# Fadi987/PL-BERT

Hardware: AMD Instinct MI355X
Metric: phoneme-tokens/sec (higher is better)
Workload: dtype bf16; 1 GPU; PL-BERT masked-phoneme training step (fwd+loss+bwd+allreduce+AdamW), ALBERT hidden 768 / 12 shared layers / FFN 2048 / 12 heads, seq_len 512, batch 32 per GPU; global_batch=32, seq_len=512, parallelism=dp1

## Files before the change

plbert_amd/_lib.py:

```python
from __future__ import annotations

import ctypes as C
import os

import torch

HERE = os.path.dirname(os.path.abspath(__file__))
LIB_PATH = os.environ.get("PLBERT_HIP_LIB") or os.path.join(HERE, "libplbert_hip.so")

PLB_PARAM_NAMES = [
    "encoder.embeddings.word_embeddings.weight",
    "encoder.embeddings.position_embeddings.weight",
    "encoder.embeddings.token_type_embeddings.weight",
    "encoder.embeddings.LayerNorm.weight",
    "encoder.embeddings.LayerNorm.bias",
    "encoder.encoder.embedding_hidden_mapping_in.weight",
    "encoder.encoder.embedding_hidden_mapping_in.bias",
    "encoder.encoder.albert_layer_groups.0.albert_layers.0.full_layer_layer_norm.weight",
    "encoder.encoder.albert_layer_groups.0.albert_layers.0.full_layer_layer_norm.bias",
    "encoder.encoder.albert_layer_groups.0.albert_layers.0.attention.query.weight",
    "encoder.encoder.albert_layer_groups.0.albert_layers.0.attention.key.weight",
    "encoder.encoder.albert_layer_groups.0.albert_layers.0.attention.value.weight",
    "encoder.encoder.albert_layer_groups.0.albert_layers.0.attention.query.bias",
    "encoder.encoder.albert_layer_groups.0.albert_layers.0.attention.key.bias",
# ... 41 lines not shown
        ("ln_eps", C.c_float), ("ln_xchg", C.c_void_p), ("ln_err", C.c_void_p), ("ln_fault", C.c_int),
    ]


class PlbGemmTN(C.Structure):
    _fields_ = [
        ("A", C.c_void_p), ("lda", C.c_int), ("Ncols", C.c_int), ("B", C.c_void_p), ("ldb", C.c_int),
        ("Mtot", C.c_int), ("N", C.c_int), ("K", C.c_int), ("rows_per_split", C.c_int), ("splits", C.c_int),
        ("slab", C.c_void_p), ("deq_a", C.c_void_p), ("deq_b", C.c_void_p),
    ]


class PlbAttn(C.Structure):
    _fields_ = [
        ("qkv", C.c_void_p), ("ldqkv", C.c_int), ("lengths", C.c_void_p),
        ("B", C.c_int), ("S", C.c_int), ("NH", C.c_int), ("H", C.c_int), ("scale", C.c_float),
        ("ctx", C.c_void_p), ("ldctx", C.c_int), ("lse", C.c_void_p),
        ("dctx", C.c_void_p), ("lddctx", C.c_int), ("delta", C.c_void_p), ("dqkv", C.c_void_p), ("lddqkv", C.c_int),
        ("colpart", C.c_void_p), ("colpart_accumulate", C.c_int),
        ("ctx8", C.c_void_p), ("ldctx8", C.c_int), ("ctx_scale", C.c_void_p), ("ctx_amax", C.c_void_p),
        ("dqkv8", C.c_void_p), ("lddqkv8", C.c_int), ("dqkv_scale", C.c_void_p), ("dqkv_amax", C.c_void_p),
        ("qoff", C.c_void_p), ("q", C.c_void_p), ("ldq", C.c_int), ("nq_total", C.c_int), ("dq", C.c_void_p), ("lddq", C.c_int),
        ("dq8", C.c_void_p), ("lddq8", C.c_int),
        ("row_start", C.c_void_p),
    ]


class PlbEmbed(C.Structure):
    _fields_ = [
        ("ids", C.c_void_p), ("T", C.c_int), ("S", C.c_int), ("E", C.c_int), ("V", C.c_int),
        ("word", C.c_void_p), ("pos", C.c_void_p), ("type0", C.c_void_p), ("gamma", C.c_void_p), ("beta", C.c_void_p),
        ("eps", C.c_float), ("out", C.c_void_p), ("ldo", C.c_int), ("dout", C.c_void_p), ("lddo", C.c_int),
        ("dx", C.c_void_p), ("dword", C.c_void_p), ("dpos", C.c_void_p), ("partials", C.c_void_p), ("nblocks", C.c_int),
        ("row_start", C.c_void_p), ("lengths", C.c_void_p), ("B", C.c_int), ("fill_slots", C.c_int),
    ]


class PlbPacking(C.Structure):
    _fields_ = [("row_start", C.c_void_p), ("rows", C.c_int32), ("used", C.c_int32)]


class PlbLayerOutputs(C.Structure):
    _fields_ = [("hidden_states", C.c_void_p), ("attentions", C.c_void_p)]


class PlbMaskedReport(C.Structure):
    _fields_ = [
        ("pred", C.c_void_p), ("rank", C.c_void_p), ("nll", C.c_void_p), ("topk_ids", C.c_void_p), ("topk_logprob", C.c_void_p),
        ("logits", C.c_void_p), ("sample_loss", C.c_void_p), ("sample_top1", C.c_void_p), ("sample_topk", C.c_void_p),
        ("totals", C.c_void_p), ("token_totals", C.c_void_p),
    ]


class PlbTokenReport(C.Structure):
    _fields_ = [
        ("topk_ids", C.c_void_p), ("topk_logprob", C.c_void_p), ("lse", C.c_void_p), ("target_logprob", C.c_void_p),
        ("target_pos", C.c_void_p), ("logits", C.c_void_p), ("totals", C.c_void_p),
    ]


class PlbLayerNorm(C.Structure):
    _fields_ = [
        ("x", C.c_void_p), ("ldx", C.c_int), ("gamma", C.c_void_p), ("beta", C.c_void_p), ("eps", C.c_float),
        ("y", C.c_void_p), ("ldy", C.c_int), ("mean", C.c_void_p), ("rstd", C.c_void_p),
        ("T", C.c_int), ("H", C.c_int), ("Tzero", C.c_int),
        ("dy", C.c_void_p), ("lddy", C.c_int), ("dx", C.c_void_p), ("lddx", C.c_int),
# ... 231 lines not shown
```

plbert_amd/csrc/embed.hip:

```cpp
#include "common.h"
#include "plbert_kernels.h"
#include "row_common.h"

namespace {
template <bool BWD>
__global__ __launch_bounds__(256) void embed_kernel(PlbEmbed p) {
  const int lane = threadIdx.x & 63, wave = threadIdx.x >> 6;
  const int E = p.E;
  const int c = lane * 4;
  const bool act = c < E;
  float4 g4 = make_float4(0, 0, 0, 0), b4 = g4, ty = g4;
  if (act) {
    g4 = *(const float4*)(p.gamma + c);
    b4 = *(const float4*)(p.beta + c);
    ty = *(const float4*)(p.type0 + c);
  }
  float dg[4] = {0, 0, 0, 0}, db[4] = {0, 0, 0, 0};
  const float invE = 1.0f / (float)E;
  for (int t = blockIdx.x * 4 + wave; t < p.T; t += gridDim.x * 4) {
    int src = t, s = 0;
    if (p.row_start) {
      int b;
      const bool owned = packed_locate(p.row_start, p.lengths, p.B, p.S, t, &b, &s);
      if (!owned && !(!BWD && p.fill_slots && s < p.S && t < p.row_start[b + 1])) {
// ... 52 lines not shown
    __shared__ float red[4][2][256];
    if (act) {
#pragma unroll
      for (int j = 0; j < 4; ++j) { red[wave][0][c + j] = dg[j]; red[wave][1][c + j] = db[j]; }
    }
    __syncthreads();
    for (int i = threadIdx.x; i < 2 * E; i += 256) {
      const int which = i / E, col = i % E;
      p.partials[(size_t)blockIdx.x * 2 * E + i] =
          red[0][which][col] + red[1][which][col] + red[2][which][col] + red[3][which][col];
    }
  }
}
}
extern "C" int plb_launch_embed_fwd(const PlbEmbed* p, hipStream_t stream) {
  if (p->E % 4 || p->E > 256 || p->T <= 0) return 1;
  if (p->row_start && (!p->lengths || p->B < 1)) return 1;
  int blocks = (p->T + 3) / 4; if (blocks > 2048) blocks = 2048;
  ProfScope ps(PLB_K_EMBED_FWD, stream, 0, (double)p->T * (8 + 2.0 * p->E));
  hipLaunchKernelGGL((embed_kernel<false>), dim3(blocks), dim3(256), 0, stream, *p);
  return LAUNCH_OK();
}
extern "C" int plb_launch_embed_bwd(const PlbEmbed* p, hipStream_t stream) {
  if (p->E % 4 || p->E > 256 || p->T <= 0 || p->nblocks <= 0) return 1;
  if (p->row_start && (!p->lengths || p->B < 1)) return 1;
  ProfScope ps(PLB_K_EMBED_BWD, stream, 0, (double)p->T * (8 + 2.0 * p->E + 8.0 * p->E));
  hipLaunchKernelGGL((embed_kernel<true>), dim3(p->nblocks), dim3(256), 0, stream, *p);
  return LAUNCH_OK();
}

namespace {
constexpr int EMB_CHUNK = 32768;
template <bool PACKED>
__global__ __launch_bounds__(256) void embed_scatter_kernel(PlbEmbed p, int P) {
  extern __shared__ int list[];
  __shared__ int wcnt[4];
  __shared__ float4 part[256];
  const int E = p.E, T = PACKED ? p.B * p.S : p.T;
  const int row = blockIdx.x;
  const int EQ = E >> 2;
  const int q = threadIdx.x % EQ, grp = threadIdx.x / EQ, ngrp = 256 / EQ;
  float4 s = make_float4(0.f, 0.f, 0.f, 0.f);
  auto add = [&](int t) {
    const float4 v = *(const float4*)(p.dx + (size_t)t * E + 4 * q);
    s.x += v.x; s.y += v.y; s.z += v.z; s.w += v.w;
  };
  if (row < p.V) {
    const int w = threadIdx.x >> 6, lane = threadIdx.x & 63;
    const int chunk = T < EMB_CHUNK ? T : EMB_CHUNK;
    const int cap = (chunk + 3) / 4 + 64;
    for (int c0 = 0; c0 < T && row != 0; c0 += EMB_CHUNK) {
      const int c1 = c0 + EMB_CHUNK < T ? c0 + EMB_CHUNK : T;
      int cnt = 0;
      for (int t0 = c0 + w * 64; t0 < c1; t0 += 256) {
        const int t = t0 + lane;
        bool hit = t < c1 && p.ids[t] == row;
        int trow = t;
        if (PACKED && hit) {
          const int b = t / p.S, sp = t - b * p.S;
          hit = sp < max(p.lengths[b], 1);
          trow = p.row_start[b] + sp;
        }
        const unsigned long long m = __builtin_amdgcn_ballot_w64(hit);
        if (hit) list[w * cap + cnt + __builtin_popcountll(m & ((1ull << lane) - 1ull))] = trow;
        cnt += __builtin_popcountll(m);
      }
      if (lane == 0) wcnt[w] = cnt;
      __syncthreads();
      for (int ww = 0; ww < 4; ++ww) {
        const int n = wcnt[ww];
        const int* l = list + ww * cap;
        int i = grp;
        for (; i + 7 * ngrp < n; i += 8 * ngrp) {
          float4 v[8];
#pragma unroll
          for (int k = 0; k < 8; ++k) v[k] = *(const float4*)(p.dx + (size_t)l[i + k * ngrp] * E + 4 * q);
          s.x += ((v[0].x + v[1].x) + (v[2].x + v[3].x)) + ((v[4].x + v[5].x) + (v[6].x + v[7].x));
          s.y += ((v[0].y + v[1].y) + (v[2].y + v[3].y)) + ((v[4].y + v[5].y) + (v[6].y + v[7].y));
          s.z += ((v[0].z + v[1].z) + (v[2].z + v[3].z)) + ((v[4].z + v[5].z) + (v[6].z + v[7].z));
          s.w += ((v[0].w + v[1].w) + (v[2].w + v[3].w)) + ((v[4].w + v[5].w) + (v[6].w + v[7].w));
        }
        for (; i + 3 * ngrp < n; i += 4 * ngrp) {
          const int t0 = l[i], t1 = l[i + ngrp], t2 = l[i + 2 * ngrp], t3 = l[i + 3 * ngrp];
          const float4 v0 = *(const float4*)(p.dx + (size_t)t0 * E + 4 * q), v1 = *(const float4*)(p.dx + (size_t)t1 * E + 4 * q);
          const float4 v2 = *(const float4*)(p.dx + (size_t)t2 * E + 4 * q), v3 = *(const float4*)(p.dx + (size_t)t3 * E + 4 * q);
          s.x += (v0.x + v1.x) + (v2.x + v3.x); s.y += (v0.y + v1.y) + (v2.y + v3.y);
          s.z += (v0.z + v1.z) + (v2.z + v3.z); s.w += (v0.w + v1.w) + (v2.w + v3.w);
        }
        for (; i < n; i += ngrp) add(l[i]);
      }
      __syncthreads();
    }
  } else {
    const int sidx = row - p.V;
    if (sidx < p.S) {
      if (PACKED) {
        for (int b = grp; b < p.B; b += ngrp)
          if (sidx < max(p.lengths[b], 1)) add(p.row_start[b] + sidx);
      } else {
        for (int t = sidx + grp * p.S; t < T; t += ngrp * p.S) add(t);
      }
    }
  }
  part[threadIdx.x] = s;
  __syncthreads();
  if (grp == 0) {
    for (int g = 1; g < ngrp; ++g) {
      const float4 v = part[g * EQ + q];
      s.x += v.x; s.y += v.y; s.z += v.z; s.w += v.w;
    }
    if (row < p.V) *(float4*)(p.dword + (size_t)row * E + 4 * q) = s;
    else if (row - p.V < P) *(float4*)(p.dpos + (size_t)(row - p.V) * E + 4 * q) = s;
  }
}
}
extern "C" int plb_launch_embed_scatter(const PlbEmbed* p, int P, hipStream_t stream) {
  if ((p->E != 64 && p->E != 128 && p->E != 256) || p->T <= 0) return 1;
  ProfScope ps(PLB_K_EMBED_BWD, stream, 0, (double)p->T * p->E * 8.0);
  if (p->row_start && (!p->lengths || p->B < 1)) return 1;
  const int Tscan = p->row_start ? p->B * p->S : p->T;
  const int chunk = Tscan < EMB_CHUNK ? Tscan : EMB_CHUNK;
  const size_t lds_bytes = (size_t)(((chunk + 3) / 4 + 64) * 4) * 4;
  if (p->row_start) hipLaunchKernelGGL(embed_scatter_kernel<true>, dim3(p->V + P), dim3(256), lds_bytes, stream, *p, P);
  else hipLaunchKernelGGL(embed_scatter_kernel<false>, dim3(p->V + P), dim3(256), lds_bytes, stream, *p, P);
  return LAUNCH_OK();
}
```

plbert_amd/csrc/engine.cpp:

```cpp
#include <stdarg.h>

#include <new>

#include "engine_internal.h"

static thread_local char g_err[512] = "";
int fail(const char* fmt, ...) {
  va_list ap;
  va_start(ap, fmt);
  vsnprintf(g_err, sizeof(g_err), fmt, ap);
  va_end(ap);
  return 1;
}
extern "C" const char* plb_last_error(void) { return g_err; }

static void layout_params(PlbEngine* e) {
  const int64_t V = e->V, E = e->E, H = e->H, I = e->I, P = e->P, NP = e->NP, NT = e->NT;
  int64_t sz[PLB_NPARAM];
  sz[PLB_WORD_EMB] = V * E; sz[PLB_POS_EMB] = P * E; sz[PLB_TYPE_EMB] = (int64_t)e->c.type_vocab_size * E;
  sz[PLB_EMB_LN_W] = E; sz[PLB_EMB_LN_B] = E;
  sz[PLB_MAP_W] = H * E; sz[PLB_MAP_B] = H;
  sz[PLB_LN2_W] = H; sz[PLB_LN2_B] = H;
  sz[PLB_Q_W] = sz[PLB_K_W] = sz[PLB_V_W] = H * H;
  sz[PLB_Q_B] = sz[PLB_K_B] = sz[PLB_V_B] = H;
// ... 92 lines not shown
    e->o_dpre1 = cv.take(L * Tp * H * 2);
    e->o_du = cv.take(L * Tp * I * 2);
    e->o_dpre2 = cv.take(L * Tp * H * 2);
    e->o_dy0 = cv.take(Tp * H * 2); e->o_dy1 = cv.take(Tp * H * 2);
    e->o_da = cv.take(Tp * H * 2); e->o_dctx = cv.take(Tp * H * 2);
    e->o_de = cv.take(Tp * E * 2);
  }
  const int64_t NM = e->NMcap;
  e->o_hm = cv.take(NM * H * 2);
  e->o_logm = cv.take(NM * 256 * 4);
  e->o_dlog = cv.take(NM * 256 * 2);
  e->o_rows = cv.take(NM * 4); e->o_tgt = cv.take(NM * 4); e->o_w = cv.take(NM * 4); e->o_lrows = cv.take(NM * 4);
  if (tr) {
    e->o_dhm = cv.take(NM * H * 2);
    int64_t slab = 0;
    {
      const int64_t Mtot = L * Tp;
      const int ntp = (int)rup(e->NT, 256);
      const int shapes[7][2] = {{(int)(3 * H), (int)H}, {(int)H, (int)H}, {(int)I, (int)H}, {(int)H, (int)I}, {(int)H, (int)E}, {e->NP, (int)H}, {ntp, (int)H}};
      for (int i = 0; i < (e->NT ? 7 : 6); ++i) {
        int rps;
        const int64_t mt = i < 4 ? Mtot : Tp;
        const int s = tn_splits(mt, shapes[i][0], shapes[i][1], &rps);
        const int64_t f = (int64_t)s * shapes[i][0] * shapes[i][1];
        if (f > slab) slab = f;
      }
    }
    e->slab_floats = slab;
    e->o_slab = cv.take(slab * 4);
    e->o_part1 = cv.take(L * e->part_rows * 3 * H * 4);
    e->o_part2 = cv.take(L * e->part_rows * 3 * H * 4);
    e->o_parte = cv.take((int64_t)e->emb_blocks * 2 * E * 4);
    e->o_dxe = cv.take(Tp * E * 4);
    e->o_ducol = cv.take(L * (2 * Tp / 128) * I * 4);
    e->qkvcol_rows = c.max_batch * ((c.max_seq + 127) / 128) * 4;
    e->o_qkvcol = cv.take((int64_t)L * e->qkvcol_rows * 3 * H * 4);
    e->o_scratch = cv.take(512 * (3 * H > I ? 3 * H : I) * 4);
    e->o_scratch2 = cv.take(512 * (3 * H > I ? 3 * H : I) * 4);
    {
      int rps;
      const int s2 = tn_splits(Tp, (int)H, (int)E, &rps);
      e->slab2_floats = (int64_t)s2 * H * E;
      e->o_slab2 = cv.take(e->slab2_floats * 4);
    }
  }
  if (e->NT) {
    const int64_t NTp = rup(e->NT, 256);
    e->NTp = (int)NTp;
    e->o_bt = cv.take(NTp * 4);
    e->o_tlrows = cv.take(Tp * 4);
    e->o_tpmax = cv.take(Tp * (NTp / 256) * 4);
    e->o_tpsum = cv.take(Tp * (NTp / 256) * 4);
    e->o_ttl = cv.take(Tp * 4); e->o_tlse = cv.take(Tp * 4); e->o_tw = cv.take(Tp * 4);
    e->o_ttgt = cv.take(Tp * 8);
    e->o_tloss = cv.take(256);
    if (tr) {
      e->o_wtT = cv.take(rup(H, 128) * NTp * 2);
      e->o_tdl = cv.take(Tp * NTp * 2);
      e->o_tscr = cv.take(32 * NTp * 4);
      e->o_tcolp = cv.take(2 * (Tp / 128) * NTp * 4);
      e->o_tgrad = cv.take(NTp * H * 4);
    }
  }
  e->o_x8 = cv.take(Ls * Tp * H); e->o_a8 = cv.take(Ls * Tp * H); e->o_g8 = cv.take(Ls * Tp * I); e->o_c8 = cv.take(Ls * Tp * H);
  e->o_wq8 = cv.take(rup(3 * H, 128) * H + 256 * H);
  e->o_wd8 = cv.take(rup(H, 128) * H + 256 * H);
// ... 260 lines not shown
```

plbert_amd/csrc/engine_calls.cpp:

```cpp
#include "engine_internal.h"

void drop_stash(PlbEngine* e, const char* by) {
  if (e && e->stash_live) { e->stash_live = false; e->stash_dead_by = by; }
}

void drop_final(PlbEngine* e, const char* by) {
  if (e) { e->fin_live = false; e->fin_dead_by = by; }
}
static void note_final(PlbEngine* e, const bf16_t* x, int B, int S, const Rows& rw) {
  e->fin_live = true; e->fin_x = x; e->fin_B = B; e->fin_S = S;
  e->fin_rows = rw.Tp; e->fin_used = rw.T; e->fin_row_start = rw.row_start;
}

static int check_shape(const PlbEngine* e, int B, int S, const char* who) {
  if (!e || !e->ws) return fail("%s: engine not bound", who);
  if (B < 1 || S < 1 || B > e->c.max_batch || S > e->c.max_seq || (int64_t)B * S > (int64_t)e->c.max_batch * e->c.max_seq)
    return fail("%s: batch %d x seq %d exceeds the engine capacity %d x %d", who, B, S, e->c.max_batch, e->c.max_seq);
  return 0;
}

static Rows padded_rows(int B, int S) { return Rows{nullptr, B * S, rup(B * S, 128)}; }
static int pick_rows(PlbEngine* e, const PlbPacking* pk, const int32_t* lengths, bool padded, int B, int S, const char* who,
                     Rows* out) {
  *out = padded_rows(B, S);
// ... 205 lines not shown
}

static int backward_tail_streams(PlbEngine* e, const int64_t* masked_ids, const int32_t* lengths, bf16_t* dy, int B, int S,
                                 const Rows& rw, int du_rows, hipStream_t s, hipStream_t s2, float* scratch2) {
  const int E = e->E, H = e->H, I = e->I, L = e->L;
  const int T = rw.T;
  const int64_t Tp = rw.Tp;
  const int64_t Mtot = (int64_t)L * Tp;
  const int64_t Mtot_c = e->pruned_rows ? (int64_t)(L - 1) * Tp + e->pruned_rows : Mtot;
  const Slots st = slots(e, Tp, B, S, 0, true, e->part_rows_used, du_rows);
  const int64_t qkvcol_all = (int64_t)L * qkvcol_rows(B, S);
  bf16_t* evec = e->at<bf16_t>(e->o_e);
  bf16_t* de = e->at<bf16_t>(e->o_de);
  PlbGemmNT g = nt_desc(dy, e->at<bf16_t>(e->o_winT), Tp, E, H);
  g.C = de; g.ldc = E;
  HB_R(s2, dy, Tp * H * 2, "dX of application 0"); HB_W(s2, de, Tp * E * 2, "dE (map-in backward)");
  TRY(plb_launch_gemm_nt(&g, 0, 0, s2));
  HB_W(s2, e->at<float>(s2 != s ? e->o_slab2 : e->o_slab), (s2 != s ? e->slab2_floats : e->slab_floats) * 4, "map-in weight-gradient slab");
  HB_W(s2, e->grd(PLB_MAP_W), e->psize[PLB_MAP_W] * 4, "map-in weight gradient");
  if (weight_grad(e, dy, H, H, evec, E, Tp, H, E, e->grd(PLB_MAP_W), s2, s2 != s)) return 1;
  HB_W(s2, scratch2, 512 * (3 * H > I ? 3 * H : I) * 4, "column-sum scratch of the side stream");
  HB_W(s2, e->grd(PLB_MAP_B), H * 4, "map-in bias gradient");
  TRY(plb_launch_colsum(dy, 1, (size_t)Tp, H, H, e->grd(PLB_MAP_B), H, 0, scratch2, 128, s2));
  HB_W(s2, e->grd(PLB_TYPE_EMB), e->psize[PLB_TYPE_EMB] * 4, "token-type embedding gradient");
  HIPTRY(hipMemsetAsync(e->grd(PLB_TYPE_EMB), 0, (size_t)e->psize[PLB_TYPE_EMB] * 4, s2));
  PlbEmbed em;
  memset(&em, 0, sizeof(em));
  em.ids = masked_ids; em.T = T; em.S = S; em.E = E; em.V = e->V;
  em.word = e->par(PLB_WORD_EMB); em.pos = e->par(PLB_POS_EMB); em.type0 = e->par(PLB_TYPE_EMB);
  em.gamma = e->par(PLB_EMB_LN_W); em.beta = e->par(PLB_EMB_LN_B); em.eps = e->c.layer_norm_eps;
  em.dout = de; em.lddo = E; em.dword = e->grd(PLB_WORD_EMB); em.dpos = e->grd(PLB_POS_EMB);
  em.dx = e->at<float>(e->o_dxe);
  em.partials = e->at<float>(e->o_parte); em.nblocks = e->emb_blocks;
  if (rw.row_start) { em.row_start = rw.row_start; em.lengths = lengths; em.B = B; }
  HB_W(s2, em.dx, Tp * E * 4, "embedding LayerNorm backward rows"); HB_W(s2, em.partials, (int64_t)e->emb_blocks * 2 * E * 4, "embedding LayerNorm partials");
  HB_W(s2, e->grd(PLB_WORD_EMB), (e->poff[PLB_MAP_W] - e->poff[PLB_WORD_EMB]) * 4, "embedding tables' and embedding LayerNorm's gradients");
  TRY(plb_launch_embed_bwd(&em, s2));
  TRY(plb_launch_embed_scatter(&em, e->P, s2));
  TRY(plb_launch_colsum(em.partials, 0, (size_t)e->emb_blocks, 2 * E, 2 * E, e->grd(PLB_EMB_LN_W), 2 * E, 0, scratch2, 1, s2));
  TRY(plb_launch_colsum(e->grd(PLB_POS_EMB), 0, (size_t)e->P, E, E, e->grd(PLB_TYPE_EMB), E, 0, scratch2, 1, s2));
  HB_R(s2, st.qkvcol, qkvcol_all * 3 * H * 4, "Q/K/V bias partial rows");
  HB_W(s2, e->grd(PLB_Q_B), 3 * H * 4, "Q/K/V bias gradients");
  TRY(plb_launch_colsum(st.qkvcol, 0, (size_t)qkvcol_all, 3 * H, 3 * H, e->grd(PLB_Q_B), 3 * H, 0, scratch2, 64, s2));
  HB_W(s2, e->grd(PLB_FFN_B), I * 4, "ffn.bias gradient");
  if (du_rows > 0) {
    HB_R(s2, st.ducol, (int64_t)L * du_rows * I * 4, "dU column-sum partial rows");
    TRY(plb_launch_colsum(st.ducol, 0, (size_t)L * du_rows, I, I, e->grd(PLB_FFN_B), I, 0, scratch2, 16, s2));
  } else {
    HB_R(s2, st.du, Mtot_c * I * 2, "dU of every application");
    TRY(plb_launch_colsum(st.du, 1, (size_t)Mtot_c, I, I, e->grd(PLB_FFN_B), I, 0, scratch2, 64, s2));
  }
  const size_t prow = (size_t)L * e->part_rows_used;
  HB_R(s2, st.part1, (int64_t)L * e->part_rows * 3 * H * 4, "LayerNorm-1 backward partial rows");
  HB_W(s2, e->grd(PLB_DENSE_B), 3 * H * 4, "dense.bias + LayerNorm-1 affine gradients");
  TRY(plb_launch_colsum(st.part1, 0, prow, 3 * H, 3 * H, e->grd(PLB_LN1_W), 2 * H, 0, scratch2, 64, s2));
  TRY(plb_launch_copy_cols(scratch2, 64, 3 * H, 2 * H, H, e->grd(PLB_DENSE_B), s2));
  HB_R(s2, st.part2, (int64_t)L * e->part_rows * 3 * H * 4, "LayerNorm-2 backward partial rows");
  HB_W(s2, e->grd(PLB_LN2_W), 2 * H * 4, "LayerNorm-2 affine gradients"); HB_W(s2, e->grd(PLB_FFNO_B), H * 4, "ffn_output.bias gradient");
  TRY(plb_launch_colsum(st.part2, 0, prow, 3 * H, 3 * H, e->grd(PLB_LN2_W), 2 * H, 0, scratch2, 64, s2));
  TRY(plb_launch_copy_cols(scratch2, 64, 3 * H, 2 * H, H, e->grd(PLB_FFNO_B), s2));
  if (s2 != s) HIPTRY(ev_record(e, e->ev_join, s2));
  const bool ov = overlapping(e);
  const bool t8 = e->tn8_call;
  float* const slab = e->at<float>(e->o_slab);
  HB_W(s, slab, e->slab_floats * 4, "weight-gradient slab"); HB_W(s, e->grd(PLB_Q_W), 3 * H * H * 4, "Q/K/V weight gradients");
  if (t8 ? weight_grad8(e, st.dq8, st.x8, Mtot, 3 * H, H, F8_DQ, F8_X, e->grd(PLB_Q_W), s)
         : weight_grad(e, st.dqkv, 3 * H, 3 * H, st.x, H, Mtot, 3 * H, H, e->grd(PLB_Q_W), s)) return 1;
  if (ov && reduce_pieces(e, kPieceQkvW, kPieceFfnW, s)) return 1;
  HB_W(s, slab, e->slab_floats * 4, "weight-gradient slab"); HB_W(s, e->grd(PLB_FFN_W), (int64_t)I * H * 4, "ffn.weight gradient");
  if (t8 ? weight_grad8(e, st.du8, st.a8, Mtot_c, I, H, F8_DU, F8_A, e->grd(PLB_FFN_W), s)
         : weight_grad(e, st.du, I, I, st.a, H, Mtot_c, I, H, e->grd(PLB_FFN_W), s)) return 1;
  if (ov && reduce_pieces(e, kPieceFfnW, kPieceSmall, s)) return 1;
  if (ov) {
    if (reduce_pieces(e, kPieceSmall, kPieceFfnoW, s2)) return 1;
  }
  HB_W(s, slab, e->slab_floats * 4, "weight-gradient slab"); HB_W(s, e->grd(PLB_FFNO_W), (int64_t)I * H * 4, "ffn_output.weight gradient");
  if (t8 ? weight_grad8(e, st.dp8, st.g8, Mtot_c, H, I, F8_DP, F8_G, e->grd(PLB_FFNO_W), s)
         : weight_grad(e, st.dpre2, H, H, st.g, I, Mtot_c, H, I, e->grd(PLB_FFNO_W), s)) return 1;
  if (ov && reduce_pieces(e, kPieceFfnoW, kPieceDenseW, s)) return 1;
  HB_W(s, slab, e->slab_floats * 4, "weight-gradient slab"); HB_W(s, e->grd(PLB_DENSE_W), (int64_t)H * H * 4, "dense.weight gradient");
// ... 246 lines not shown
```

plbert_amd/csrc/engine_internal.h:

```cpp
#pragma once
#include <hip/hip_runtime.h>
#include <stdint.h>
#include <stdio.h>
#include <stdlib.h>
#include <string.h>

#include <array>
#include <map>
#include <string>
#include <vector>

#include "../../include/plbert.h"
#include "plbert_kernels.h"

#pragma GCC visibility push(hidden)

int fail(const char* fmt, ...);

static const unsigned kStreamOrderEvent = hipEventDisableTiming | hipEventReleaseToDevice;

inline int64_t rup(int64_t x, int64_t m) { return (x + m - 1) / m * m; }

#define TRY(x)                                                                    \
  do {                                                                            \
// ... 27 lines not shown
  void record(hipEvent_t e, int st) { vc[st][st] += 1; ev[e] = vc[st]; }
  void wait(int st, hipEvent_t e);
  void access(int st, const void* p, size_t bytes, bool wr, const char* what);
  void new_call() { log.clear(); waits = 0; }
};

struct PlbEngine {
  PlbConfig c;
  int64_t poff[PLB_NPARAM], psize[PLB_NPARAM], ptotal, ptrain;
  int E, H, I, L, NH, V, P, NP, NT;
  int64_t Tcap;
  int64_t NMcap;
  int NTp = 0;
  bool infer = false;
  int qkvcol_rows = 0;
  int64_t slab2_floats;
  int64_t slab_floats;
  int64_t ws_bytes;
  int ln_blocks, emb_blocks;
  int part_rows = 0;
  int ln_fuse = 3;
  int64_t lnx_bytes = 0;
  bool gelu_dstash_on = true;
  bool fp8_tn = true;
  int f8n = 0;
  bool packed_dual = false;
  bool packed_fp8 = false;
  int64_t o_wbf, o_wqkvT, o_wdT, o_w1T, o_w2T, o_wpT, o_winT;
  int64_t o_e, o_x, o_qkv, o_ctx, o_pre1, o_a, o_u, o_g, o_pre2;
  int64_t o_lse, o_delta, o_mean1, o_rstd1, o_mean2, o_rstd2;
  int64_t o_dqkv, o_dpre1, o_du, o_dpre2;
  int64_t o_dy0, o_dy1, o_da, o_dctx, o_de;
  int64_t o_hm, o_logm, o_dlog, o_dhm, o_rows, o_tgt, o_w, o_lrows;
  int64_t o_slab, o_part1, o_part2, o_parte, o_scratch, o_dxe, o_ducol, o_slab2, o_scratch2, o_qkvcol = 0;
  int64_t o_lnx = 0, o_lnerr = 0;
  int64_t o_rep_rank = 0, o_rep_nll = 0, o_rep_tok = 0;
  int64_t o_tr_rows = 0, o_tr_tgt = 0, o_tr_scratch = 0;
  int64_t o_bt = 0, o_wtT = 0, o_tdl = 0, o_tlrows = 0, o_tscr = 0, o_tgrad = 0, o_tloss = 0;
  int64_t o_tpmax = 0, o_tpsum = 0, o_ttl = 0, o_tlse = 0, o_tw = 0, o_ttgt = 0, o_tcolp = 0;
  int64_t o_x8 = 0, o_a8 = 0, o_g8 = 0, o_c8 = 0, o_dp8 = 0, o_du8 = 0, o_dp18 = 0, o_dq8 = 0;
  int64_t o_wq8 = 0, o_wd8 = 0, o_w18 = 0, o_w28 = 0, o_w2T8 = 0, o_w1T8 = 0, o_wqT8 = 0, o_wdT8 = 0;
  int64_t o_f8amax = 0, o_f8scale = 0, o_f8deq = 0, o_f8stats = 0;
  bool fp8_on = false, fp8_ready = false, fp8_bwd_ready = false, fp8_wstale = true;
  bool u_is_derivative = false;
  bool tn8_call = false;
  int part_rows_used = 0;
  int pruned_rows = 0;
  int64_t last_app_rows[2] = {0, 0};
  int64_t last_exec_rows[2] = {0, 0};
  bool tok_grads_live = false;
  bool head_grads_live = true;
  bool tok_pad_zeroed = false;
  int tok_steps = 0;
  bool rep_valid = false, rep_dual = false;
  int rep_n = 0, rep_B = 0;
  int64_t rep_tok_rows = 0;
  bool fin_live = false;
  const char* fin_dead_by = "no call has run the encoder on this engine since plb_bind";
  const bf16_t* fin_x = nullptr;
  int fin_B = 0, fin_S = 0;
  int64_t fin_rows = 0, fin_used = 0;
  const int32_t* fin_row_start = nullptr;
  float* accum = nullptr;
  bool grads_fresh = false;
  bool win_open = false;
  const char* win_closed_by = "no FIRST add has opened one";
  bool win_head = false, win_tok = false;
// ... 132 lines not shown
```

plbert_amd/csrc/plbert_kernels.h:

```cpp
#pragma once
#include <hip/hip_runtime.h>
#include <stdint.h>

typedef uint16_t bf16_t;

extern "C" {

enum PlbKernelClass {
  PLB_K_GEMM_NT = 0, PLB_K_GEMM_NT_GELU, PLB_K_GEMM_NT_GELUBWD, PLB_K_GEMM_NT_F32, PLB_K_GEMM_TN,
  PLB_K_ATTN_FWD, PLB_K_ATTN_BWD_DQ, PLB_K_ATTN_BWD_DKV, PLB_K_LN_FWD, PLB_K_LN_BWD, PLB_K_EMBED_FWD,
  PLB_K_EMBED_BWD, PLB_K_COLSUM, PLB_K_REDUCE, PLB_K_ROWS, PLB_K_CE, PLB_K_ADAMW, PLB_K_CAST, PLB_K_TOKEN_CE, PLB_K_GEMM_NT_CE, PLB_K_GEMM_NT_SMALL, PLB_K_FP8, PLB_K_ATTN_BWD,
  PLB_K_GEMM_NT_FP8, PLB_K_GEMM_NT_GELU_FP8, PLB_K_GEMM_NT_GELUBWD_FP8,
  PLB_K_GEMM_NT_LNFWD, PLB_K_GEMM_NT_LNBWD,
  PLB_K_GEMM_NT_LNFWD_FP8, PLB_K_GEMM_NT_LNBWD_FP8, PLB_K_GEMM_TN_FP8,
  PLB_K_NCLASS
};
int plb_prof_begin(int cls, hipStream_t s, double flops, double bytes);
void plb_prof_end(int tok, hipStream_t s);

typedef struct {
  const bf16_t* A; int lda;
  const bf16_t* B; int ldb;
  int M, N, K;
  int Mstore;
// ... 29 lines not shown
int plb_launch_gemm_nt_fp8_gelud(const PlbGemmNT* p, int backward, int a_bf8, hipStream_t stream);
int plb_gemm_nt_fp8_gelud_tile_rows(int M);
int plb_ln_fault_take(void);
int plb_launch_gemm_nt(const PlbGemmNT* p, int act, int out_f32, hipStream_t stream);
int plb_launch_gemm_nt_big(const PlbGemmNT* p, int tile, int act, int out_f32, hipStream_t stream);
int plb_gemm_nt_colpart_rows(int M, int N, int K);
void plb_set_gemm_nt_tile(int tile);
void plb_set_gemm_nt_prefetch(int on);

typedef struct {
  const bf16_t* A; int lda; int Ncols;
  const bf16_t* B; int ldb;
  int Mtot, N, K;
  int rows_per_split, splits;
  float* slab;
  const float* deq_a; const float* deq_b;
} PlbGemmTN;
int plb_launch_gemm_tn(const PlbGemmTN* p, hipStream_t stream);
int plb_launch_gemm_tn_fp8(const PlbGemmTN* p, hipStream_t stream);
int plb_launch_gemm_tn_big(const PlbGemmTN* p, hipStream_t stream);

int plb_launch_reduce_slabs(const float* slab, int splits, size_t n, float* out, int accumulate, hipStream_t stream);

typedef struct {
  const int64_t* ids; int T, S, E, V;
  const float *word, *pos, *type0, *gamma, *beta;
  float eps;
  bf16_t* out; int ldo;
  const bf16_t* dout; int lddo;
  float* dx;
  float *dword, *dpos;
  float* partials;
  int nblocks;
  const int32_t* row_start; const int32_t* lengths; int B; int fill_slots;
} PlbEmbed;
int plb_launch_embed_fwd(const PlbEmbed* p, hipStream_t stream);
int plb_launch_embed_bwd(const PlbEmbed* p, hipStream_t stream);
int plb_launch_embed_scatter(const PlbEmbed* p, int P, hipStream_t stream);

typedef struct {
  const bf16_t* x; int ldx;
  const float *gamma, *beta; float eps;
  bf16_t* y; int ldy;
  float *mean, *rstd;
  int T, H;
  int Tzero;
  const bf16_t* dy; int lddy;
  bf16_t* dx; int lddx;
  float* partials; int nblocks;
  int accumulate;
  uint8_t* out8; int ld8; const float* q_scale; float* q_amax;
} PlbLayerNorm;
int plb_launch_amax(const void* x, int is_bf16, size_t rows, int cols, int ld, float* amax, hipStream_t stream);
int plb_launch_fp8_scales(float* amax, float* scale, float* deq, int n, float fmax, int group, hipStream_t stream);
int plb_launch_fp8_scales2(float* amax, float* scale, float* deq, int n, float fmax, int group, int n2, float fmax2,
                           float* stats, int hist_from, hipStream_t stream);
int plb_launch_quantize(const void* x, int is_bf16, size_t rows, int cols, int ld, const float* scale, uint8_t* out, int ldo,
                        int bf8, hipStream_t stream);
int plb_launch_quantize_multi(int n, const void* const* src, const int* is_bf16, const size_t* elements,
                              const float* const* scale, uint8_t* const* dst, float* const* amax, hipStream_t stream);
int plb_launch_ln_fwd(const PlbLayerNorm* p, hipStream_t stream);
int plb_launch_ln_bwd(const PlbLayerNorm* p, hipStream_t stream);

int plb_launch_colsum(const void* X, int is_bf16, size_t R, int N, int ld, float* out, int Nout, int accumulate,
                      float* scratch, int nsplit, hipStream_t stream);

int plb_launch_copy_cols(const float* scratch, int nsplit, int N, int col0, int Nout, float* out, hipStream_t stream);

// ... 121 lines not shown
```

plbert_amd/csrc/reduce.hip:

```cpp
#include "common.h"
#include "plbert_kernels.h"
#include "row_common.h"

namespace {
template <bool BF16>
__global__ __launch_bounds__(256) void colsum_kernel(const void* X, size_t R, int N, int ld, float* scratch, int nsplit) {
  __shared__ float red[8][256];
  const int tid = threadIdx.x;
  const int rsub = tid >> 5, cl = tid & 31;
  const int c = blockIdx.x * 256 + cl * 8;
  const size_t rows_per = (R + nsplit - 1) / nsplit;
  const size_t r0 = (size_t)blockIdx.y * rows_per;
  size_t r1 = r0 + rows_per; if (r1 > R) r1 = R;
  float acc[8] = {0, 0, 0, 0, 0, 0, 0, 0};
  if (c < N) {
    size_t r = r0 + rsub;
    if (BF16) {
      const bf16_t* px = (const bf16_t*)X + c;
      for (; r + 24 < r1; r += 32) {
        uint4 u0 = *(const uint4*)(px + r * ld), u1 = *(const uint4*)(px + (r + 8) * ld);
        uint4 u2 = *(const uint4*)(px + (r + 16) * ld), u3 = *(const uint4*)(px + (r + 24) * ld);
        acc[0] += (bf_lo(u0.x) + bf_lo(u1.x)) + (bf_lo(u2.x) + bf_lo(u3.x));
        acc[1] += (bf_hi(u0.x) + bf_hi(u1.x)) + (bf_hi(u2.x) + bf_hi(u3.x));
        acc[2] += (bf_lo(u0.y) + bf_lo(u1.y)) + (bf_lo(u2.y) + bf_lo(u3.y));
        acc[3] += (bf_hi(u0.y) + bf_hi(u1.y)) + (bf_hi(u2.y) + bf_hi(u3.y));
        acc[4] += (bf_lo(u0.z) + bf_lo(u1.z)) + (bf_lo(u2.z) + bf_lo(u3.z));
        acc[5] += (bf_hi(u0.z) + bf_hi(u1.z)) + (bf_hi(u2.z) + bf_hi(u3.z));
        acc[6] += (bf_lo(u0.w) + bf_lo(u1.w)) + (bf_lo(u2.w) + bf_lo(u3.w));
        acc[7] += (bf_hi(u0.w) + bf_hi(u1.w)) + (bf_hi(u2.w) + bf_hi(u3.w));
      }
    }
    if (!BF16) {
      const float* px = (const float*)X + c;
      for (; r + 24 < r1; r += 32) {
        const float* q0 = px + r * ld;
        const float* q1 = px + (r + 8) * ld;
        const float* q2 = px + (r + 16) * ld;
        const float* q3 = px + (r + 24) * ld;
        const float4 a0 = *(const float4*)q0, b0 = *(const float4*)(q0 + 4), a1 = *(const float4*)q1, b1 = *(const float4*)(q1 + 4);
        const float4 a2 = *(const float4*)q2, b2 = *(const float4*)(q2 + 4), a3 = *(const float4*)q3, b3 = *(const float4*)(q3 + 4);
        acc[0] += (a0.x + a1.x) + (a2.x + a3.x); acc[1] += (a0.y + a1.y) + (a2.y + a3.y);
        acc[2] += (a0.z + a1.z) + (a2.z + a3.z); acc[3] += (a0.w + a1.w) + (a2.w + a3.w);
        acc[4] += (b0.x + b1.x) + (b2.x + b3.x); acc[5] += (b0.y + b1.y) + (b2.y + b3.y);
        acc[6] += (b0.z + b1.z) + (b2.z + b3.z); acc[7] += (b0.w + b1.w) + (b2.w + b3.w);
      }
    }
    for (; r < r1; r += 8) {
      if (BF16) {
        uint4 u = *(const uint4*)((const bf16_t*)X + r * ld + c);
        acc[0] += bf_lo(u.x); acc[1] += bf_hi(u.x); acc[2] += bf_lo(u.y); acc[3] += bf_hi(u.y);
        acc[4] += bf_lo(u.z); acc[5] += bf_hi(u.z); acc[6] += bf_lo(u.w); acc[7] += bf_hi(u.w);
      } else {
        const float* px = (const float*)X + r * ld + c;
        float4 a = *(const float4*)px, b = *(const float4*)(px + 4);
        acc[0] += a.x; acc[1] += a.y; acc[2] += a.z; acc[3] += a.w;
        acc[4] += b.x; acc[5] += b.y; acc[6] += b.z; acc[7] += b.w;
      }
    }
  }
#pragma unroll
  for (int j = 0; j < 8; ++j) red[rsub][cl * 8 + j] = acc[j];
  __syncthreads();
  const int col = blockIdx.x * 256 + tid;
  if (col < N) {
    float s = 0.f;
#pragma unroll
    for (int k = 0; k < 8; ++k) s += red[k][tid];
    scratch[(size_t)blockIdx.y * N + col] = s;
  }
}

__global__ __launch_bounds__(256) void reduce_cols_kernel(const float* scratch, int nsplit, int N, int Nout, float* out,
                                                          int accumulate, int col0) {
  __shared__ float red[8][32];
  const int c = threadIdx.x & 31, g = threadIdx.x >> 5;
  const int j = blockIdx.x * 32 + c;
  float s0 = 0.f, s1 = 0.f, s2 = 0.f, s3 = 0.f;
  if (j < Nout) {
    const float* px = scratch + col0 + j;
    int k = g;
    for (; k + 24 < nsplit; k += 32) {
      s0 += px[(size_t)k * N]; s1 += px[(size_t)(k + 8) * N]; s2 += px[(size_t)(k + 16) * N]; s3 += px[(size_t)(k + 24) * N];
    }
    for (; k < nsplit; k += 8) s0 += px[(size_t)k * N];
  }
  red[g][c] = (s0 + s1) + (s2 + s3);
  __syncthreads();
  if (g == 0 && j < Nout) {
    const float t = ((red[0][c] + red[1][c]) + (red[2][c] + red[3][c])) + ((red[4][c] + red[5][c]) + (red[6][c] + red[7][c]));
    out[j] = accumulate ? out[j] + t : t;
  }
}
}
extern "C" int plb_launch_colsum(const void* X, int is_bf16, size_t R, int N, int ld, float* out, int Nout,
                                 int accumulate, float* scratch, int nsplit, hipStream_t stream) {
  if (N % 8 || ld % 8 || nsplit <= 0 || Nout > N) return 1;
  ProfScope ps(PLB_K_COLSUM, stream, 0, (double)R * N * (is_bf16 ? 2 : 4));
  dim3 grid((N + 255) / 256, nsplit);
  if (is_bf16) hipLaunchKernelGGL((colsum_kernel<true>), grid, dim3(256), 0, stream, X, R, N, ld, scratch, nsplit);
  else hipLaunchKernelGGL((colsum_kernel<false>), grid, dim3(256), 0, stream, X, R, N, ld, scratch, nsplit);
  if (hipGetLastError() != hipSuccess) return 2;
  hipLaunchKernelGGL(reduce_cols_kernel, dim3((unsigned)((Nout + 31) / 32)), dim3(256), 0, stream, scratch, nsplit, N,
                     Nout, out, accumulate, 0);
  return LAUNCH_OK();
}
extern "C" int plb_launch_copy_cols(const float* scratch, int nsplit, int N, int col0, int Nout, float* out,
                                    hipStream_t stream) {
  if (nsplit <= 0 || col0 < 0 || col0 + Nout > N) return 1;
  hipLaunchKernelGGL(reduce_cols_kernel, dim3((unsigned)((Nout + 31) / 32)), dim3(256), 0, stream, scratch, nsplit, N,
                     Nout, out, 0, col0);
  return LAUNCH_OK();
}

namespace {
__global__ __launch_bounds__(256) void reduce_slabs_kernel(const float* slab, int splits, size_t n, float* out, int accumulate) {
  const size_t i = ((size_t)blockIdx.x * blockDim.x + threadIdx.x) * 4;
  if (i >= n) return;
  if (i + 4 <= n) {
    float4 s = accumulate ? *(const float4*)(out + i) : make_float4(0, 0, 0, 0);
    int k = 0;
    for (; k + 4 <= splits; k += 4) {
      const float4 v0 = *(const float4*)(slab + (size_t)k * n + i), v1 = *(const float4*)(slab + (size_t)(k + 1) * n + i);
      const float4 v2 = *(const float4*)(slab + (size_t)(k + 2) * n + i), v3 = *(const float4*)(slab + (size_t)(k + 3) * n + i);
      s.x = (((s.x + v0.x) + v1.x) + v2.x) + v3.x; s.y = (((s.y + v0.y) + v1.y) + v2.y) + v3.y;
      s.z = (((s.z + v0.z) + v1.z) + v2.z) + v3.z; s.w = (((s.w + v0.w) + v1.w) + v2.w) + v3.w;
    }
    for (; k < splits; ++k) {
      float4 v = *(const float4*)(slab + (size_t)k * n + i);
      s.x += v.x; s.y += v.y; s.z += v.z; s.w += v.w;
// ... 45 lines not shown
```

Baseline: 1.703 million tokens/s.

## Split embedding scatter over token ranges and widen column-sum parallelism

The word-embedding gradient scatter now splits each vocabulary row's token scan into 1024-token ranges. Each range runs in its own block and writes a partial row, and a new kernel sums the partials into dword. This gives a small vocabulary far more blocks than one block per row. The column-sum kernel is generalized so fp32 rows use 4 columns per lane with deeper unrolling, and several colsum calls get larger split counts. The cost is an extra partial buffer and an extra reduction launch.

```diff
diff --git a/plbert_amd/_lib.py b/plbert_amd/_lib.py
--- a/plbert_amd/_lib.py
+++ b/plbert_amd/_lib.py
@@ -97,6 +97,7 @@
         ("word", C.c_void_p), ("pos", C.c_void_p), ("type0", C.c_void_p), ("gamma", C.c_void_p), ("beta", C.c_void_p),
         ("eps", C.c_float), ("out", C.c_void_p), ("ldo", C.c_int), ("dout", C.c_void_p), ("lddo", C.c_int),
         ("dx", C.c_void_p), ("dword", C.c_void_p), ("dpos", C.c_void_p), ("partials", C.c_void_p), ("nblocks", C.c_int),
+        ("wrange", C.c_int), ("wpart", C.c_void_p),
         ("row_start", C.c_void_p), ("lengths", C.c_void_p), ("B", C.c_int), ("fill_slots", C.c_int),
     ]
 
diff --git a/plbert_amd/csrc/embed.hip b/plbert_amd/csrc/embed.hip
--- a/plbert_amd/csrc/embed.hip
+++ b/plbert_amd/csrc/embed.hip
@@ -108,12 +108,14 @@
 namespace {
 constexpr int EMB_CHUNK = 32768;
 template <bool PACKED>
-__global__ __launch_bounds__(256) void embed_scatter_kernel(PlbEmbed p, int P) {
+__global__ __launch_bounds__(256) void embed_scatter_kernel(PlbEmbed p, int P, int nranges, int range) {
   extern __shared__ int list[];
   __shared__ int wcnt[4];
   __shared__ float4 part[256];
   const int E = p.E, T = PACKED ? p.B * p.S : p.T;
-  const int row = blockIdx.x;
+  const int nw = p.V * nranges;
+  const int row = (int)blockIdx.x < nw ? (int)blockIdx.x / nranges : p.V + ((int)blockIdx.x - nw);
+  const int rg = (int)blockIdx.x < nw ? (int)blockIdx.x % nranges : 0;
   const int EQ = E >> 2;
   const int q = threadIdx.x % EQ, grp = threadIdx.x / EQ, ngrp = 256 / EQ;
   float4 s = make_float4(0.f, 0.f, 0.f, 0.f);
@@ -123,10 +125,14 @@
   };
   if (row < p.V) {
     const int w = threadIdx.x >> 6, lane = threadIdx.x & 63;
-    const int chunk = T < EMB_CHUNK ? T : EMB_CHUNK;
+    const int tb = nranges > 1 ? rg * range : 0;
+    const int te = nranges > 1 && tb + range < T ? tb + range : T;
+    const int span = nranges > 1 ? range : T;
+    const int chunk = span < EMB_CHUNK ? span : EMB_CHUNK;
     const int cap = (chunk + 3) / 4 + 64;
-    for (int c0 = 0; c0 < T && row != 0; c0 += EMB_CHUNK) {
-      const int c1 = c0 + EMB_CHUNK < T ? c0 + EMB_CHUNK : T;
+    if (nranges > 1 && row == 0) return;
+    for (int c0 = tb; c0 < te && row != 0; c0 += EMB_CHUNK) {
+      const int c1 = c0 + EMB_CHUNK < te ? c0 + EMB_CHUNK : te;
       int cnt = 0;
       for (int t0 = c0 + w * 64; t0 < c1; t0 += 256) {
         const int t = t0 + lane;
@@ -147,15 +153,6 @@
         const int n = wcnt[ww];
         const int* l = list + ww * cap;
         int i = grp;
-        for (; i + 7 * ngrp < n; i += 8 * ngrp) {
-          float4 v[8];
-#pragma unroll
-          for (int k = 0; k < 8; ++k) v[k] = *(const float4*)(p.dx + (size_t)l[i + k * ngrp] * E + 4 * q);
-          s.x += ((v[0].x + v[1].x) + (v[2].x + v[3].x)) + ((v[4].x + v[5].x) + (v[6].x + v[7].x));
-          s.y += ((v[0].y + v[1].y) + (v[2].y + v[3].y)) + ((v[4].y + v[5].y) + (v[6].y + v[7].y));
-          s.z += ((v[0].z + v[1].z) + (v[2].z + v[3].z)) + ((v[4].z + v[5].z) + (v[6].z + v[7].z));
-          s.w += ((v[0].w + v[1].w) + (v[2].w + v[3].w)) + ((v[4].w + v[5].w) + (v[6].w + v[7].w));
-        }
         for (; i + 3 * ngrp < n; i += 4 * ngrp) {
           const int t0 = l[i], t1 = l[i + ngrp], t2 = l[i + 2 * ngrp], t3 = l[i + 3 * ngrp];
           const float4 v0 = *(const float4*)(p.dx + (size_t)t0 * E + 4 * q), v1 = *(const float4*)(p.dx + (size_t)t1 * E + 4 * q);
@@ -185,19 +182,52 @@
       const float4 v = part[g * EQ + q];
       s.x += v.x; s.y += v.y; s.z += v.z; s.w += v.w;
     }
-    if (row < p.V) *(float4*)(p.dword + (size_t)row * E + 4 * q) = s;
+    if (row < p.V) *(float4*)((nranges > 1 ? p.wpart + ((size_t)row * nranges + rg) * E : p.dword + (size_t)row * E) + 4 * q) = s;
     else if (row - p.V < P) *(float4*)(p.dpos + (size_t)(row - p.V) * E + 4 * q) = s;
   }
+}
+__global__ __launch_bounds__(256) void embed_ranges_sum_kernel(const float* wpart, int V, int E, int nranges, float* dword) {
+  const int EQ = E >> 2;
+  const size_t i = (size_t)blockIdx.x * 256 + threadIdx.x;
+  if (i >= (size_t)V * EQ) return;
+  const int v = (int)(i / EQ), q = (int)(i % EQ);
+  float4 s = make_float4(0.f, 0.f, 0.f, 0.f);
+  if (v != 0) {
+    const float* px = wpart + (size_t)v * nranges * E + 4 * q;
+    int r = 0;
+    for (; r + 8 <= nranges; r += 8) {
+      float4 u[8];
+#pragma unroll
+      for (int k = 0; k < 8; ++k) u[k] = *(const float4*)(px + (size_t)(r + k) * E);
+#pragma unroll
+      for (int k = 0; k < 8; ++k) { s.x += u[k].x; s.y += u[k].y; s.z += u[k].z; s.w += u[k].w; }
+    }
+    for (; r < nranges; ++r) {
+      const float4 u = *(const float4*)(px + (size_t)r * E);
+      s.x += u.x; s.y += u.y; s.z += u.z; s.w += u.w;
+    }
+  }
+  *(float4*)(dword + (size_t)v * E + 4 * q) = s;
 }
 }
 extern "C" int plb_launch_embed_scatter(const PlbEmbed* p, int P, hipStream_t stream) {
   if ((p->E != 64 && p->E != 128 && p->E != 256) || p->T <= 0) return 1;
   ProfScope ps(PLB_K_EMBED_BWD, stream, 0, (double)p->T * p->E * 8.0);
   if (p->row_start && (!p->lengths || p->B < 1)) return 1;
+  if (p->wpart && p->wrange <= 0) return 1;
   const int Tscan = p->row_start ? p->B * p->S : p->T;
-  const int chunk = Tscan < EMB_CHUNK ? Tscan : EMB_CHUNK;
+  int nranges = p->wpart ? (Tscan + p->wrange - 1) / p->wrange : 1;
+  const int span = nranges > 1 ? p->wrange : Tscan;
+  const int chunk = span < EMB_CHUNK ? span : EMB_CHUNK;
   const size_t lds_bytes = (size_t)(((chunk + 3) / 4 + 64) * 4) * 4;
-  if (p->row_start) hipLaunchKernelGGL(embed_scatter_kernel<true>, dim3(p->V + P), dim3(256), lds_bytes, stream, *p, P);
-  else hipLaunchKernelGGL(embed_scatter_kernel<false>, dim3(p->V + P), dim3(256), lds_bytes, stream, *p, P);
+  const dim3 grid((unsigned)(p->V * nranges + P));
+  if (p->row_start) hipLaunchKernelGGL(embed_scatter_kernel<true>, grid, dim3(256), lds_bytes, stream, *p, P, nranges, span);
+  else hipLaunchKernelGGL(embed_scatter_kernel<false>, grid, dim3(256), lds_bytes, stream, *p, P, nranges, span);
+  if (nranges > 1) {
+    if (hipGetLastError() != hipSuccess) return 2;
+    const size_t n4 = (size_t)p->V * (p->E / 4);
+    hipLaunchKernelGGL(embed_ranges_sum_kernel, dim3((unsigned)((n4 + 255) / 256)), dim3(256), 0, stream, p->wpart, p->V, p->E,
+                       nranges, p->dword);
+  }
   return LAUNCH_OK();
 }
diff --git a/plbert_amd/csrc/engine.cpp b/plbert_amd/csrc/engine.cpp
--- a/plbert_amd/csrc/engine.cpp
+++ b/plbert_amd/csrc/engine.cpp
@@ -148,6 +148,7 @@
     e->o_part2 = cv.take(L * e->part_rows * 3 * H * 4);
     e->o_parte = cv.take((int64_t)e->emb_blocks * 2 * E * 4);
     e->o_dxe = cv.take(Tp * E * 4);
+    e->o_wparte = cv.take((int64_t)e->V * ((T + PLB_EMB_RANGE - 1) / PLB_EMB_RANGE) * E * 4);
     e->o_ducol = cv.take(L * (2 * Tp / 128) * I * 4);
     e->qkvcol_rows = c.max_batch * ((c.max_seq + 127) / 128) * 4;
     e->o_qkvcol = cv.take((int64_t)L * e->qkvcol_rows * 3 * H * 4);
diff --git a/plbert_amd/csrc/engine_calls.cpp b/plbert_amd/csrc/engine_calls.cpp
--- a/plbert_amd/csrc/engine_calls.cpp
+++ b/plbert_amd/csrc/engine_calls.cpp
@@ -261,20 +261,23 @@
   em.dout = de; em.lddo = E; em.dword = e->grd(PLB_WORD_EMB); em.dpos = e->grd(PLB_POS_EMB);
   em.dx = e->at<float>(e->o_dxe);
   em.partials = e->at<float>(e->o_parte); em.nblocks = e->emb_blocks;
+  em.wpart = e->at<float>(e->o_wparte); em.wrange = PLB_EMB_RANGE;
   if (rw.row_start) { em.row_start = rw.row_start; em.lengths = lengths; em.B = B; }
   HB_W(s2, em.dx, Tp * E * 4, "embedding LayerNorm backward rows"); HB_W(s2, em.partials, (int64_t)e->emb_blocks * 2 * E * 4, "embedding LayerNorm partials");
   HB_W(s2, e->grd(PLB_WORD_EMB), (e->poff[PLB_MAP_W] - e->poff[PLB_WORD_EMB]) * 4, "embedding tables' and embedding LayerNorm's gradients");
+  const int64_t wpart_bytes = (int64_t)e->V * (((int64_t)B * S + PLB_EMB_RANGE - 1) / PLB_EMB_RANGE) * E * 4;
+  HB_W(s2, em.wpart, wpart_bytes, "word-row partials of the scatter's token ranges"); HB_R(s2, em.wpart, wpart_bytes, "word-row partials of the scatter's token ranges");
   TRY(plb_launch_embed_bwd(&em, s2));
   TRY(plb_launch_embed_scatter(&em, e->P, s2));
-  TRY(plb_launch_colsum(em.partials, 0, (size_t)e->emb_blocks, 2 * E, 2 * E, e->grd(PLB_EMB_LN_W), 2 * E, 0, scratch2, 1, s2));
-  TRY(plb_launch_colsum(e->grd(PLB_POS_EMB), 0, (size_t)e->P, E, E, e->grd(PLB_TYPE_EMB), E, 0, scratch2, 1, s2));
+  TRY(plb_launch_colsum(em.partials, 0, (size_t)e->emb_blocks, 2 * E, 2 * E, e->grd(PLB_EMB_LN_W), 2 * E, 0, scratch2, 64, s2));
+  TRY(plb_launch_colsum(e->grd(PLB_POS_EMB), 0, (size_t)e->P, E, E, e->grd(PLB_TYPE_EMB), E, 0, scratch2, 16, s2));
   HB_R(s2, st.qkvcol, qkvcol_all * 3 * H * 4, "Q/K/V bias partial rows");
   HB_W(s2, e->grd(PLB_Q_B), 3 * H * 4, "Q/K/V bias gradients");
   TRY(plb_launch_colsum(st.qkvcol, 0, (size_t)qkvcol_all, 3 * H, 3 * H, e->grd(PLB_Q_B), 3 * H, 0, scratch2, 64, s2));
   HB_W(s2, e->grd(PLB_FFN_B), I * 4, "ffn.bias gradient");
   if (du_rows > 0) {
     HB_R(s2, st.ducol, (int64_t)L * du_rows * I * 4, "dU column-sum partial rows");
-    TRY(plb_launch_colsum(st.ducol, 0, (size_t)L * du_rows, I, I, e->grd(PLB_FFN_B), I, 0, scratch2, 16, s2));
+    TRY(plb_launch_colsum(st.ducol, 0, (size_t)L * du_rows, I, I, e->grd(PLB_FFN_B), I, 0, scratch2, 96, s2));
   } else {
     HB_R(s2, st.du, Mtot_c * I * 2, "dU of every application");
     TRY(plb_launch_colsum(st.du, 1, (size_t)Mtot_c, I, I, e->grd(PLB_FFN_B), I, 0, scratch2, 64, s2));
diff --git a/plbert_amd/csrc/engine_internal.h b/plbert_amd/csrc/engine_internal.h
--- a/plbert_amd/csrc/engine_internal.h
+++ b/plbert_amd/csrc/engine_internal.h
@@ -83,7 +83,7 @@
   int64_t o_dqkv, o_dpre1, o_du, o_dpre2;
   int64_t o_dy0, o_dy1, o_da, o_dctx, o_de;
   int64_t o_hm, o_logm, o_dlog, o_dhm, o_rows, o_tgt, o_w, o_lrows;
-  int64_t o_slab, o_part1, o_part2, o_parte, o_scratch, o_dxe, o_ducol, o_slab2, o_scratch2, o_qkvcol = 0;
+  int64_t o_slab, o_part1, o_part2, o_parte, o_wparte, o_scratch, o_dxe, o_ducol, o_slab2, o_scratch2, o_qkvcol = 0;
   int64_t o_lnx = 0, o_lnerr = 0;
   int64_t o_rep_rank = 0, o_rep_nll = 0, o_rep_tok = 0;
   int64_t o_tr_rows = 0, o_tr_tgt = 0, o_tr_scratch = 0;
diff --git a/plbert_amd/csrc/plbert_kernels.h b/plbert_amd/csrc/plbert_kernels.h
--- a/plbert_amd/csrc/plbert_kernels.h
+++ b/plbert_amd/csrc/plbert_kernels.h
@@ -85,8 +85,11 @@
   float *dword, *dpos;
   float* partials;
   int nblocks;
+  int wrange;
+  float* wpart;
   const int32_t* row_start; const int32_t* lengths; int B; int fill_slots;
 } PlbEmbed;
+#define PLB_EMB_RANGE 1024
 int plb_launch_embed_fwd(const PlbEmbed* p, hipStream_t stream);
 int plb_launch_embed_bwd(const PlbEmbed* p, hipStream_t stream);
 int plb_launch_embed_scatter(const PlbEmbed* p, int P, hipStream_t stream);
diff --git a/plbert_amd/csrc/reduce.hip b/plbert_amd/csrc/reduce.hip
--- a/plbert_amd/csrc/reduce.hip
+++ b/plbert_amd/csrc/reduce.hip
@@ -4,68 +4,64 @@
 
 namespace {
 template <bool BF16>
+DEVI float cs_el(const uint4& u, int j) {
+  const uint32_t w[4] = {u.x, u.y, u.z, u.w};
+  if (BF16) return (j & 1) ? bf_hi(w[j >> 1]) : bf_lo(w[j >> 1]);
+  return __uint_as_float(w[j]);
+}
+template <bool BF16>
 __global__ __launch_bounds__(256) void colsum_kernel(const void* X, size_t R, int N, int ld, float* scratch, int nsplit) {
-  __shared__ float red[8][256];
+  constexpr int CPL = BF16 ? 8 : 4;
+  constexpr int LPR = 256 / CPL;
+  constexpr int RL = 256 / LPR;
+  constexpr int ES = BF16 ? 2 : 4;
+  __shared__ float red[RL][256];
   const int tid = threadIdx.x;
-  const int rsub = tid >> 5, cl = tid & 31;
-  const int c = blockIdx.x * 256 + cl * 8;
+  const int rsub = tid / LPR, cl = tid % LPR;
+  const int c = blockIdx.x * 256 + cl * CPL;
   const size_t rows_per = (R + nsplit - 1) / nsplit;
   const size_t r0 = (size_t)blockIdx.y * rows_per;
   size_t r1 = r0 + rows_per; if (r1 > R) r1 = R;
-  float acc[8] = {0, 0, 0, 0, 0, 0, 0, 0};
+  float acc[CPL];
+#pragma unroll
+  for (int j = 0; j < CPL; ++j) acc[j] = 0.f;
   if (c < N) {
+    const size_t rowb = (size_t)ld * ES;
+    const char* px = (const char*)X + (size_t)c * ES;
     size_t r = r0 + rsub;
-    if (BF16) {
-      const bf16_t* px = (const bf16_t*)X + c;
-      for (; r + 24 < r1; r += 32) {
-        uint4 u0 = *(const uint4*)(px + r * ld), u1 = *(const uint4*)(px + (r + 8) * ld);
-        uint4 u2 = *(const uint4*)(px + (r + 16) * ld), u3 = *(const uint4*)(px + (r + 24) * ld);
-        acc[0] += (bf_lo(u0.x) + bf_lo(u1.x)) + (bf_lo(u2.x) + bf_lo(u3.x));
-        acc[1] += (bf_hi(u0.x) + bf_hi(u1.x)) + (bf_hi(u2.x) + bf_hi(u3.x));
-        acc[2] += (bf_lo(u0.y) + bf_lo(u1.y)) + (bf_lo(u2.y) + bf_lo(u3.y));
-        acc[3] += (bf_hi(u0.y) + bf_hi(u1.y)) + (bf_hi(u2.y) + bf_hi(u3.y));
-        acc[4] += (bf_lo(u0.z) + bf_lo(u1.z)) + (bf_lo(u2.z) + bf_lo(u3.z));
-        acc[5] += (bf_hi(u0.z) + bf_hi(u1.z)) + (bf_hi(u2.z) + bf_hi(u3.z));
-        acc[6] += (bf_lo(u0.w) + bf_lo(u1.w)) + (bf_lo(u2.w) + bf_lo(u3.w));
-        acc[7] += (bf_hi(u0.w) + bf_hi(u1.w)) + (bf_hi(u2.w) + bf_hi(u3.w));
-      }
+    for (; r + 7 * RL < r1; r += 8 * RL) {
+      const char* q = px + r * rowb;
+      uint4 u[8];
+#pragma unroll
+      for (int k = 0; k < 8; ++k) u[k] = *(const uint4*)(q + (size_t)(k * RL) * rowb);
+#pragma unroll
+      for (int j = 0; j < CPL; ++j)
+        acc[j] += ((cs_el<BF16>(u[0], j) + cs_el<BF16>(u[1], j)) + (cs_el<BF16>(u[2], j) + cs_el<BF16>(u[3], j))) +
+                  ((cs_el<BF16>(u[4], j) + cs_el<BF16>(u[5], j)) + (cs_el<BF16>(u[6], j) + cs_el<BF16>(u[7], j)));
     }
-    if (!BF16) {
-      const float* px = (const float*)X + c;
-      for (; r + 24 < r1; r += 32) {
-        const float* q0 = px + r * ld;
-        const float* q1 = px + (r + 8) * ld;
-        const float* q2 = px + (r + 16) * ld;
-        const float* q3 = px + (r + 24) * ld;
-        const float4 a0 = *(const float4*)q0, b0 = *(const float4*)(q0 + 4), a1 = *(const float4*)q1, b1 = *(const float4*)(q1 + 4);
-        const float4 a2 = *(const float4*)q2, b2 = *(const float4*)(q2 + 4), a3 = *(const float4*)q3, b3 = *(const float4*)(q3 + 4);
-        acc[0] += (a0.x + a1.x) + (a2.x + a3.x); acc[1] += (a0.y + a1.y) + (a2.y + a3.y);
-        acc[2] += (a0.z + a1.z) + (a2.z + a3.z); acc[3] += (a0.w + a1.w) + (a2.w + a3.w);
-        acc[4] += (b0.x + b1.x) + (b2.x + b3.x); acc[5] += (b0.y + b1.y) + (b2.y + b3.y);
-        acc[6] += (b0.z + b1.z) + (b2.z + b3.z); acc[7] += (b0.w + b1.w) + (b2.w + b3.w);
-      }
+    for (; r + 3 * RL < r1; r += 4 * RL) {
+      const char* q = px + r * rowb;
+      uint4 u[4];
+#pragma unroll
+      for (int k = 0; k < 4; ++k) u[k] = *(const uint4*)(q + (size_t)(k * RL) * rowb);
+#pragma unroll
+      for (int j = 0; j < CPL; ++j)
+        acc[j] += (cs_el<BF16>(u[0], j) + cs_el<BF16>(u[1], j)) + (cs_el<BF16>(u[2], j) + cs_el<BF16>(u[3], j));
     }
-    for (; r < r1; r += 8) {
-      if (BF16) {
-        uint4 u = *(const uint4*)((const bf16_t*)X + r * ld + c);
-        acc[0] += bf_lo(u.x); acc[1] += bf_hi(u.x); acc[2] += bf_lo(u.y); acc[3] += bf_hi(u.y);
-        acc[4] += bf_lo(u.z); acc[5] += bf_hi(u.z); acc[6] += bf_lo(u.w); acc[7] += bf_hi(u.w);
-      } else {
-        const float* px = (const float*)X + r * ld + c;
-        float4 a = *(const float4*)px, b = *(const float4*)(px + 4);
-        acc[0] += a.x; acc[1] += a.y; acc[2] += a.z; acc[3] += a.w;
-        acc[4] += b.x; acc[5] += b.y; acc[6] += b.z; acc[7] += b.w;
-      }
+    for (; r < r1; r += RL) {
+      const uint4 u = *(const uint4*)(px + r * rowb);
+#pragma unroll
+      for (int j = 0; j < CPL; ++j) acc[j] += cs_el<BF16>(u, j);
     }
   }
 #pragma unroll
-  for (int j = 0; j < 8; ++j) red[rsub][cl * 8 + j] = acc[j];
+  for (int j = 0; j < CPL; ++j) red[rsub][cl * CPL + j] = acc[j];
   __syncthreads();
   const int col = blockIdx.x * 256 + tid;
   if (col < N) {
-    float s = 0.f;
+    float s = red[0][tid];
 #pragma unroll
-    for (int k = 0; k < 8; ++k) s += red[k][tid];
+    for (int k = 1; k < RL; ++k) s += red[k][tid];
     scratch[(size_t)blockIdx.y * N + col] = s;
   }
 }
@@ -75,16 +71,23 @@
   __shared__ float red[8][32];
   const int c = threadIdx.x & 31, g = threadIdx.x >> 5;
   const int j = blockIdx.x * 32 + c;
-  float s0 = 0.f, s1 = 0.f, s2 = 0.f, s3 = 0.f;
+  float s = 0.f;
   if (j < Nout) {
     const float* px = scratch + col0 + j;
     int k = g;
+    for (; k + 56 < nsplit; k += 64) {
+      float v[8];
+#pragma unroll
+      for (int i = 0; i < 8; ++i) v[i] = px[(size_t)(k + 8 * i) * N];
+      s += ((v[0] + v[1]) + (v[2] + v[3])) + ((v[4] + v[5]) + (v[6] + v[7]));
+    }
     for (; k + 24 < nsplit; k += 32) {
-      s0 += px[(size_t)k * N]; s1 += px[(size_t)(k + 8) * N]; s2 += px[(size_t)(k + 16) * N]; s3 += px[(size_t)(k + 24) * N];
+      const float v0 = px[(size_t)k * N], v1 = px[(size_t)(k + 8) * N], v2 = px[(size_t)(k + 16) * N], v3 = px[(size_t)(k + 24) * N];
+      s += (v0 + v1) + (v2 + v3);
     }
-    for (; k < nsplit; k += 8) s0 += px[(size_t)k * N];
+    for (; k < nsplit; k += 8) s += px[(size_t)k * N];
   }
-  red[g][c] = (s0 + s1) + (s2 + s3);
+  red[g][c] = s;
   __syncthreads();
   if (g == 0 && j < Nout) {
     const float t = ((red[0][c] + red[1][c]) + (red[2][c] + red[3][c])) + ((red[4][c] + red[5][c]) + (red[6][c] + red[7][c]));
@@ -94,7 +97,7 @@
 }
 extern "C" int plb_launch_colsum(const void* X, int is_bf16, size_t R, int N, int ld, float* out, int Nout,
                                  int accumulate, float* scratch, int nsplit, hipStream_t stream) {
-  if (N % 8 || ld % 8 || nsplit <= 0 || Nout > N) return 1;
+  if (N <= 0 || ld < N || ld % (is_bf16 ? 8 : 4) || nsplit <= 0 || Nout > N || Nout < 0) return 1;
   ProfScope ps(PLB_K_COLSUM, stream, 0, (double)R * N * (is_bf16 ? 2 : 4));
   dim3 grid((N + 255) / 256, nsplit);
   if (is_bf16) hipLaunchKernelGGL((colsum_kernel<true>), grid, dim3(256), 0, stream, X, R, N, ld, scratch, nsplit);
```

New measurement: 1.708 million tokens/s (median of 6 runs). About the same (+0.3%).
